# Ye-zixiao/Double-YOLO-Kaist

Measured on AMD Instinct MI355X. Metric: paired RGB+LWIR images/sec (train step), higher is better.
Workload: dtype bf16; 1 GPU; kaist_dyolov4_fshare_global_concat_se3.cfg train step (fwd+loss+bwd+Adam), 640x512 pairs, batch 16/GPU; global_batch=16, parallelism=dp1

## Files before the change

### double-yolo-kaist_amd/csrc/conv_igemm.hip

```cpp
#include <stddef.h>
#include <string.h>
#include "dyk_common.h"

int dyk_conv_launch_n128(const DykConvDesc* d, hipStream_t s);
int dyk_conv_launch_n80(const DykConvDesc* d, hipStream_t s);
int dyk_conv_launch_n160(const DykConvDesc* d, hipStream_t s);
int dyk_conv_launch_halo(const DykConvDesc* d, hipStream_t s, int th);
int dyk_conv_launch_kg(const DykConvDesc* d, hipStream_t s);
int dyk_conv_launch_lt(const DykConvDesc* d, hipStream_t s);
int dyk_conv_launch_sc(const DykConvDesc* d, hipStream_t s);
int dyk_conv_launch_pw(const DykConvDesc* d, hipStream_t s);

static int conv_validate(const DykConvDesc* d) {
    if (!d || !d->x || !d->w || !d->y) return DYK_ERR_ARG;
    if (d->ntaps < 0 || d->ntaps > DYK_MAX_TAPS) return DYK_ERR_ARG;
    if (d->B <= 0 || d->Hg <= 0 || d->Wg <= 0 || d->Cout <= 0 || d->Cin <= 0) return DYK_ERR_ARG;
    if (d->ncls < 0 || d->ncls > 4) return DYK_ERR_ARG;
    for (int c = 0; c < (d->ncls > 1 ? d->ncls : 0); ++c)
        if (d->cls_first[c] < 0 || d->cls_ntaps[c] < 0 || d->cls_first[c] + d->cls_ntaps[c] > d->ntaps || d->cls_ooy[c] < 0 ||
            d->cls_ooy[c] >= d->osy || d->cls_oox[c] < 0 || d->cls_oox[c] >= d->osx)
            return DYK_ERR_ARG;
    if (d->dtype == DYK_F16 && (d->flags & (DYK_EPI_STATS | DYK_EPI_BNFWD | DYK_EPI_BNBWD | DYK_EPI_ADDEND))) return DYK_ERR_UNSUPPORTED;
    if ((d->flags & DYK_EPI_STATS) && !d->stats) return DYK_ERR_ARG;
    if ((d->flags & DYK_EPI_RESIDUAL) && !d->res) return DYK_ERR_ARG;
    if ((d->flags & DYK_EPI_ADDEND) && (!(d->flags & DYK_EPI_BNBWD) || ((uintptr_t)d->add % 16))) return DYK_ERR_ARG;
    if (d->flags & DYK_EPI_BNFWD) {
        if (!(d->flags & DYK_EPI_STATS) || (d->flags & (DYK_EPI_AFFINE | DYK_EPI_ACCUM | DYK_EPI_OUT_F32 | DYK_EPI_BNBWD | DYK_EPI_ADDEND)))
            return DYK_ERR_ARG;
        if (d->dtype != DYK_BF16 || d->twin || d->ncls > 1 || d->bn_count <= 0) return DYK_ERR_ARG;
        if (!d->y2 || !d->bn_counter || !d->scale || !d->shift || ((uintptr_t)d->y2 % 16) || ((uintptr_t)d->bn_counter % 8)) return DYK_ERR_ARG;
        if (d->Cout % 8 || d->ldy % 8 || d->ldy2 % 8 || d->ldy2 < d->Cout) return DYK_ERR_ARG;
        if ((d->flags & DYK_EPI_RESIDUAL) && (d->ldr % 4 || ((uintptr_t)d->res % 8))) return DYK_ERR_ARG;
        if ((long)d->B * d->Ho * d->Wo * d->ldy2 >= (1L << 31)) return DYK_ERR_ARG;
    }
    if (d->flags & DYK_EPI_BNBWD) {
        if (d->flags & (DYK_EPI_AFFINE | DYK_EPI_RESIDUAL | DYK_EPI_STATS | DYK_EPI_ACCUM | DYK_EPI_OUT_F32)) return DYK_ERR_ARG;
        if (!d->res || !d->stats || !d->scale || !d->shift || !d->aux0 || !d->aux1) return DYK_ERR_ARG;
        const int es = d->dtype == DYK_F32 ? 4 : 2;
        if (d->Cout % (16 / es) || ((size_t)d->ldy * es) % 16 || ((size_t)d->ldr * es) % 16 || ((uintptr_t)d->y % 16) ||
            ((uintptr_t)d->res % 16))
            return DYK_ERR_ARG;
    }
    if (d->splitk > 1) {
        if (d->splitk > 16 || !d->sk_ws || !d->sk_cnt || ((uintptr_t)d->sk_ws % 16) || ((uintptr_t)d->sk_cnt % 4) || d->sk_cnt_n <= 0 ||
            d->sk_ws_bytes <= 0)
            return DYK_ERR_ARG;
        if (d->twin || d->ncls > 1 || (d->flags & DYK_EPI_BNFWD)) return DYK_ERR_ARG;
    }
    if (d->dtype != DYK_BF16 && d->dtype != DYK_F32 && d->dtype != DYK_F16) return DYK_ERR_ARG;
    const int epv = d->dtype == DYK_F32 ? 4 : 8;
    if (d->ldx % epv || ((uintptr_t)d->x % 16) || ((uintptr_t)d->w % 16)) return DYK_ERR_ARG;
    if ((long)d->B * d->Hi * d->Wi * d->ldx >= (1L << 31)) return DYK_ERR_ARG;
    if ((long)d->B * d->Ho * d->Wo * d->ldy >= (1L << 31)) return DYK_ERR_ARG;
    if (d->Hi > 16000 || d->Wi > 16000) return DYK_ERR_ARG;
    return DYK_OK;
}

extern "C" int dyk_conv_igemm(const DykConvDesc* d, void* stream) {
    int rc0 = conv_validate(d);
    if (rc0 != DYK_OK) return rc0;
    if (d->twin) {
        if ((rc0 = conv_validate(d->twin)) != DYK_OK) return rc0;
        const size_t lo = offsetof(DykConvDesc, dtype), hi = offsetof(DykConvDesc, twin);
        if (memcmp((const char*)d + lo, (const char*)d->twin + lo, hi - lo) != 0) return DYK_ERR_ARG;
    }
    hipStream_t s = (hipStream_t)stream;
    const int tile = d->dtype != DYK_F32 ? (d->tune >> 12) & 0xf : 0;
    if (d->flags & DYK_EPI_BNFWD) {
        if (tile == 1 || tile == 3) return dyk_conv_launch_n80(d, s);
        if (tile == 2 || tile == 4) return dyk_conv_launch_n160(d, s);
        return dyk_conv_launch_n128(d, s);
    }
    if (tile == 5) {
        const int rc = dyk_conv_launch_lt(d, s);
        if (rc != DYK_ERR_UNSUPPORTED || ((d->tune >> 23) & 1)) return rc;
        return dyk_conv_launch_n160(d, s);
    }
    if (tile == 6) {
        const int rc = (d->splitk > 1 || d->dtype != DYK_BF16) ? DYK_ERR_UNSUPPORTED : dyk_conv_launch_sc(d, s);
        if (rc != DYK_ERR_UNSUPPORTED || ((d->tune >> 23) & 1)) return rc;
        return dyk_conv_launch_n128(d, s);
    }
    if (tile == 7) {
        const int rc = dyk_conv_launch_pw(d, s);
        if (rc != DYK_ERR_UNSUPPORTED || ((d->tune >> 23) & 1)) return rc;
        return dyk_conv_launch_n128(d, s);
    }
    if (((d->tune >> 28) & 7) == 1) {
        const int rc = dyk_conv_launch_kg(d, s);
        if (rc != DYK_ERR_UNSUPPORTED || ((d->tune >> 23) & 1)) return rc;
    }
    if (tile == 3 || tile == 4) {
        const int rc = dyk_conv_launch_halo(d, s, tile == 3 ? 4 : 8);
        if (rc != DYK_ERR_UNSUPPORTED || ((d->tune >> 23) & 1)) return rc;
        return tile == 3 ? dyk_conv_launch_n80(d, s) : dyk_conv_launch_n160(d, s);
    }
    if (tile == 1) return dyk_conv_launch_n80(d, s);
    if (tile == 2) return dyk_conv_launch_n160(d, s);
    return dyk_conv_launch_n128(d, s);
}

extern "C" int dyk_conv_bnfwd_max_grid(void) { return 256; }

extern "C" int dyk_conv_grid(const DykConvDesc* d) {
    if (!d || d->B <= 0 || d->Hg <= 0 || d->Wg <= 0 || d->Cout <= 0) return DYK_ERR_ARG;
    const int tile = d->dtype != DYK_F32 ? (d->tune >> 12) & 0xf : 0;
    const int bn = (tile == 1 || tile == 3) ? 80 : ((tile == 2 || tile == 4) ? 160 : 128);
    int bm = d->Cout > 64 ? 128 : (d->Cout > 32 ? 64 : 32);
    const int bm_code = (d->tune >> 24) & 0xf;
    if (bm_code >= 1 && bm_code <= 3) bm = 16 << bm_code;
    if (bn == 80 && bm == 32) bm = 64;
    const long n = (long)d->B * d->Hg * d->Wg;
    return (int)((n + bn - 1) / bn) * ((d->Cout + bm - 1) / bm) * (d->ncls > 1 ? d->ncls : 1);
}

extern "C" int64_t dyk_conv_splitk_ws_bytes(const DykConvDesc* d, int32_t* tiles) {
    if (tiles) *tiles = 0;
    if (!d || d->B <= 0 || d->Hg <= 0 || d->Wg <= 0 || d->Cout <= 0) return DYK_ERR_ARG;
    if (d->splitk <= 1) return 0;
    const long n = (long)d->B * d->Hg * d->Wg;
    const int tile = d->dtype != DYK_F32 ? (d->tune >> 12) & 0xf : 0;
    int64_t bytes = 0;
    int32_t nt = 0;
    auto cover = [&](int bm, int bn) {
        const int64_t tm = (d->Cout + bm - 1) / bm, tn = (n + bn - 1) / bn;
        const int64_t b = tm * tn * (int64_t)d->splitk * bm * bn * 4;
        if (b > bytes) bytes = b;
        if (tm * tn > nt) nt = (int32_t)(tm * tn);
    };
    {
        const int bn = (tile == 1 || tile == 3) ? 80 : ((tile == 2 || tile == 4 || tile == 5) ? 160 : 128);
        int bm = d->Cout > 64 ? 128 : (d->Cout > 32 ? 64 : 32);
        const int bm_code = (d->tune >> 24) & 0xf;
        if (tile != 5 && bm_code >= 1 && bm_code <= 3) bm = 16 << bm_code;
        if (bn == 80 && bm == 32) bm = 64;
        if (((d->tune >> 28) & 7) == 1 && bm < 64) bm = 64;
        cover(bm, bn);
    }
    if (tile == 5) {
        const int shape = (d->tune >> 8) & 0xf;
        if (shape == 1) cover(128, 320);
        else if (shape == 2) cover(256, 160);
        else cover(128, 160);
    }
    if (tiles) *tiles = nt;
    return bytes;
}
```

### double-yolo-kaist_amd/csrc/conv_sc.hip

```cpp
#include <stddef.h>
#include <string.h>
#include <type_traits>
#include "dyk_common.h"

namespace {

#define LDS_AS __attribute__((address_space(3)))
__device__ uint4 dyk_sc_zero_page[8];

struct ScArgs {
    DykConvDesc d;
    int PH, PW, npatch;
    int miny, minx;
    int tiles_y, tiles_x, ntiles;
    int tap_shift[9];
    int tap_w[9];
    int cls_first[4], cls_ntaps[4], cls_ooy[4], cls_oox[4];
};

__device__ inline void sc_glds16(const void* gsrc, unsigned lds_addr) {
    unsigned keep;
    asm volatile("s_mov_b32 %0, m0\n\ts_mov_b32 m0, %2\n\ts_nop 0\n\tglobal_load_lds_dwordx4 %1, off\n\ts_mov_b32 m0, %0"
                 : "=&s"(keep)
                 : "v"(gsrc), "s"(lds_addr)
                 : "memory");
}
__device__ inline unsigned sc_lds_addr(const void* p) {
    return __builtin_amdgcn_readfirstlane((unsigned)(size_t)(LDS_AS const char*)p);
}

constexpr int SC_M = 32, SC_TH = 8, SC_TW = 16;

template <int NCLS, int K> struct ScCfg {
    static constexpr int PITCH = K * 2;
    static constexpr int NCH = PITCH / 16;
    static constexpr int RPI = 1024 / PITCH;
    static constexpr int R256 = PITCH >= 256 ? 1 : 256 / PITCH;
    static constexpr int PROWS = NCLS == 4 ? 9 * 17 : 10 * 18;
    static constexpr int NPI = ((PROWS + RPI - 1) / RPI + 3) / 4;
    static constexpr int P_BYTES = NPI * 4 * 1024;
    static constexpr int W_BYTES = 9 * SC_M * PITCH;
    static constexpr int NWI = W_BYTES / 1024 / 4;
    static constexpr int LDS = W_BYTES + 2 * P_BYTES + 4 * 2 * SC_M * 4 + 4 * SC_M * 4;
    static_assert(W_BYTES % 4096 == 0, "weights in whole instructions per wave");
};
template <int K> __device__ inline int sc_key(int row) { return (row / ScCfg<1, K>::R256) & (ScCfg<1, K>::NCH - 1); }

template <int NCLS, int K, int ACTB>
__global__ __launch_bounds__(256) __attribute__((amdgpu_waves_per_eu(2))) void conv_sc_kernel(const ScArgs g) {
    using C = ScCfg<NCLS, K>;
    using T = bf16_t;
    constexpr int PITCH = C::PITCH, NPI = C::NPI, NWI = C::NWI, RPI = C::RPI, VPR = C::NCH;
    const DykConvDesc& a = g.d;
    extern __shared__ __attribute__((aligned(16))) char smem[];
    char* sW = smem;
    char* sP = smem + C::W_BYTES;
    float* s_stat = (float*)(smem + C::W_BYTES + 2 * C::P_BYTES);

    const int tid = threadIdx.x, lane = tid & 63;
    const int wv = __builtin_amdgcn_readfirstlane(tid >> 6);
    const int i16 = lane & 15, kq = lane >> 4;
    const T* zero = (const T*)dyk_sc_zero_page;
    const int Hi_s = __builtin_amdgcn_readfirstlane(a.Hi), Wi_s = __builtin_amdgcn_readfirstlane(a.Wi);
    const int ldx_s = __builtin_amdgcn_readfirstlane(a.ldx), ldy_s = __builtin_amdgcn_readfirstlane(a.ldy), ldr_s = __builtin_amdgcn_readfirstlane(a.ldr);
    const int Ho_s = __builtin_amdgcn_readfirstlane(a.Ho), Wo_s = __builtin_amdgcn_readfirstlane(a.Wo);
    const int osy = __builtin_amdgcn_readfirstlane(a.osy), osx = __builtin_amdgcn_readfirstlane(a.osx);
    const int PW = g.PW;

    {
        const T* wg = (const T*)a.w;
#pragma unroll
        for (int j = 0; j < NWI; ++j) {
            const int q = j * 4 + wv;
            const int row = q * RPI + lane / VPR, ps = lane % VPR;
            const int lc = ps ^ sc_key<K>(row);
            sc_glds16(wg + (long)row * K + lc * 8, sc_lds_addr(sW + q * 1024));
        }
    }
    int p_eoff[NPI], p_yx[NPI];
#pragma unroll
    for (int j = 0; j < NPI; ++j) {
        const int row = (j * 4 + wv) * RPI + lane / VPR, ps = lane % VPR;
        const int lc = ps ^ sc_key<K>(row);
        const int py = row / PW, px = row - py * PW;
        p_yx[j] = row < g.npatch ? (py << 16) | px : (0x7000 << 16);
        p_eoff[j] = (py * Wi_s + px) * ldx_s + lc * 8;
    }
    auto stage_patch = [&](int tile, int buf) {
        const int tx = tile % g.tiles_x, r = tile / g.tiles_x;
        const int ty = r % g.tiles_y, b = r / g.tiles_y;
        const int ys = ty * SC_TH + g.miny, xs = tx * SC_TW + g.minx;
        const T* x00 = (const T*)a.x + (long)((b * Hi_s + ys) * Wi_s + xs) * ldx_s;
        char* dst = sP + buf * C::P_BYTES;
#pragma unroll
        for (int j = 0; j < NPI; ++j) {
            const int hy = p_yx[j] >> 16, hx = p_yx[j] & 0xffff;
            const bool ok = ((unsigned)(ys + hy) < (unsigned)Hi_s) & ((unsigned)(xs + hx) < (unsigned)Wi_s);
            const T* cand = x00 + p_eoff[j];
            sc_glds16(ok ? cand : zero, sc_lds_addr(dst + (j * 4 + wv) * 1024));
        }
    };

    float* s_bn = s_stat + 4 * 2 * SC_M;
    if (tid < 4 * SC_M) {
        const int which = tid / SC_M, ch = tid % SC_M;
        const float* src = which == 0 ? a.scale : which == 1 ? a.shift : which == 2 ? a.aux0 : a.aux1;
        s_bn[tid] = src[ch];
    }
    float s1[8], s2[8];
#pragma unroll
    for (int j = 0; j < 8; ++j) s1[j] = s2[j] = 0.f;
    int pb[2];
#pragma unroll
    for (int ni = 0; ni < 2; ++ni) pb[ni] = (2 * wv + ni) * PW + i16;
    int wa[2];
#pragma unroll
    for (int mi = 0; mi < 2; ++mi) wa[mi] = (mi * 16 + i16) * PITCH;
    const int wkey[2] = {sc_key<K>(i16), sc_key<K>(16 + i16)};

    int buf = 0;
    int tile = blockIdx.x;
    if (tile < g.ntiles) stage_patch(tile, 0);
    for (; tile < g.ntiles; tile += gridDim.x) {
        asm volatile("s_waitcnt vmcnt(0)" ::: "memory");
        __builtin_amdgcn_s_barrier();
        if (tile + (int)gridDim.x < g.ntiles) stage_patch(tile + gridDim.x, buf ^ 1);
        const char* P = sP + buf * C::P_BYTES;

        const int tx = tile % g.tiles_x, rr = tile / g.tiles_x;
        const int ty = rr % g.tiles_y, b = rr / g.tiles_y;
        const int xo = (tx * SC_TW + i16) * osx;
        uint2 raw[NCLS][2][2];
        int opix[NCLS][2];
#pragma unroll
        for (int c = 0; c < NCLS; ++c)
#pragma unroll
            for (int ni = 0; ni < 2; ++ni) {
                const int yo = (ty * SC_TH + 2 * wv + ni) * osy + (NCLS > 1 ? g.cls_ooy[c] : a.ooy);
                opix[c][ni] = (b * Ho_s + yo) * Wo_s + xo + (NCLS > 1 ? g.cls_oox[c] : a.oox);
#pragma unroll
                for (int mi = 0; mi < 2; ++mi)
                    raw[c][mi][ni] = *(const uint2*)((const T*)a.res + (long)opix[c][ni] * ldr_s + mi * 16 + kq * 4);
            }

        f32x4_t acc[NCLS][2][2];
#pragma unroll
        for (int c = 0; c < NCLS; ++c)
#pragma unroll
            for (int mi = 0; mi < 2; ++mi)
#pragma unroll
                for (int ni = 0; ni < 2; ++ni) acc[c][mi][ni] = (f32x4_t){0.f, 0.f, 0.f, 0.f};
        {
            int t = 0;
#pragma unroll
            for (int c = 0; c < NCLS; ++c) {
                constexpr int NT[4] = {NCLS == 4 ? 1 : 9, 2, 2, 4};
#pragma unroll
                for (int q = 0; q < NT[c]; ++q, ++t) {
                    const int shift = g.tap_shift[t];
                    const char* Wt = sW + g.tap_w[t] * (SC_M * PITCH);
                    int prow[2], pkey[2];
#pragma unroll
                    for (int ni = 0; ni < 2; ++ni) { prow[ni] = pb[ni] + shift; pkey[ni] = sc_key<K>(prow[ni]); }
#pragma unroll
                    for (int kb = 0; kb < K / 32; ++kb) {
                        const int chunk = kq + 4 * kb;
                        bf16x8_t fa[2], fb[2];
#pragma unroll
                        for (int mi = 0; mi < 2; ++mi) fa[mi] = *(const bf16x8_t*)(Wt + wa[mi] + ((chunk ^ wkey[mi]) << 4));
#pragma unroll
                        for (int ni = 0; ni < 2; ++ni) fb[ni] = *(const bf16x8_t*)(P + prow[ni] * PITCH + ((chunk ^ pkey[ni]) << 4));
#pragma unroll
                        for (int mi = 0; mi < 2; ++mi)
#pragma unroll
                            for (int ni = 0; ni < 2; ++ni)
                                acc[c][mi][ni] = __builtin_amdgcn_mfma_f32_16x16x32_bf16(fa[mi], fb[ni], acc[c][mi][ni], 0, 0, 0);
                    }
                }
            }
        }

#pragma unroll
        for (int mi = 0; mi < 2; ++mi) {
            const f32x4_t scv = *(const f32x4_t*)(s_bn + 0 * SC_M + mi * 16 + kq * 4), shv = *(const f32x4_t*)(s_bn + 1 * SC_M + mi * 16 + kq * 4);
            const f32x4_t muv = *(const f32x4_t*)(s_bn + 2 * SC_M + mi * 16 + kq * 4), rsv = *(const f32x4_t*)(s_bn + 3 * SC_M + mi * 16 + kq * 4);
#pragma unroll
            for (int c = 0; c < NCLS; ++c)
#pragma unroll
                for (int ni = 0; ni < 2; ++ni) {
                    const f32x4_t v = acc[c][mi][ni];
                    const uint32_t g01 = f32x2_to_bf16x2(v[0], v[1]), g23 = f32x2_to_bf16x2(v[2], v[3]);
                    const uint2 y2 = raw[c][mi][ni];
                    uint32_t ow[2];
#pragma unroll
                    for (int h = 0; h < 2; ++h) {
                        const uint32_t gw = h ? g23 : g01, yw = h ? y2.y : y2.x;
                        const dyk_f32x2_t gv = {__uint_as_float(gw << 16), __uint_as_float(gw & 0xffff0000u)};
                        const dyk_f32x2_t yv = {__uint_as_float(yw << 16), __uint_as_float(yw & 0xffff0000u)};
                        const int j = mi * 4 + 2 * h;
                        const dyk_f32x2_t sc2 = {scv[2 * h], scv[2 * h + 1]}, sh2 = {shv[2 * h], shv[2 * h + 1]};
                        const dyk_f32x2_t mu2 = {muv[2 * h], muv[2 * h + 1]}, rs2 = {rsv[2 * h], rsv[2 * h + 1]};
                        const dyk_f32x2_t u = yv * sc2 + sh2;
                        const dyk_f32x2_t da = gv * act_bwd2_c<ACTB>(u, a.act);
                        const dyk_f32x2_t xh = (yv - mu2) * rs2;
                        const dyk_f32x2_t p = da * xh;
                        s1[j] += da[0]; s1[j + 1] += da[1];
                        s2[j] += p[0]; s2[j + 1] += p[1];
                        ow[h] = f32x2_to_bf16x2(da[0], da[1]);
                    }
                    *(uint2*)((T*)a.y + (long)opix[c][ni] * ldy_s + mi * 16 + kq * 4) = make_uint2(ow[0], ow[1]);
                }
        }
        buf ^= 1;
    }

#pragma unroll
    for (int j = 0; j < 8; ++j) { s1[j] = row16_sum(s1[j]); s2[j] = row16_sum(s2[j]); }
    if (i16 == 0) {
#pragma unroll
        for (int mi = 0; mi < 2; ++mi)
#pragma unroll
            for (int r = 0; r < 4; ++r) {
                s_stat[(wv * 2 + 0) * SC_M + mi * 16 + kq * 4 + r] = s1[mi * 4 + r];
                s_stat[(wv * 2 + 1) * SC_M + mi * 16 + kq * 4 + r] = s2[mi * 4 + r];
            }
    }
    __syncthreads();
    if (tid < 2 * SC_M) {
        const int ml = tid % SC_M, which = tid / SC_M;
        const float tot = (s_stat[(0 * 2 + which) * SC_M + ml] + s_stat[(1 * 2 + which) * SC_M + ml]) +
                          (s_stat[(2 * 2 + which) * SC_M + ml] + s_stat[(3 * 2 + which) * SC_M + ml]);
        double* st = a.stats + (size_t)((unsigned)blockIdx.x % (unsigned)(a.stats_slots > 0 ? a.stats_slots : 1)) * 2 * a.Cout;
        atomicAdd(st + which * a.Cout + ml, (double)tot);
    }
}

bool sc_eligible(const DykConvDesc* d) {
    if (d->dtype != DYK_BF16 || d->ntaps != 9 || d->twin) return false;
    if (d->flags != DYK_EPI_BNBWD) return false;
    if (d->Cout != SC_M || (d->Cin != 64)) return false;
    if (d->isy != 1 || d->isx != 1 || d->osy != d->osx) return false;
    if (d->Hg % SC_TH || d->Wg % SC_TW) return false;
    if (d->ldx % 8 || d->ldy % 4 || d->ldr % 4 || ((uintptr_t)d->y % 8) || ((uintptr_t)d->res % 8)) return false;
    if (d->ncls > 1) {
        if (d->ncls != 4 || d->osy != 2) return false;
        if (d->Ho != 2 * d->Hg || d->Wo != 2 * d->Wg) return false;
        static const int nt[4] = {1, 2, 2, 4};
        for (int c = 0, q = 0; c < 4; q += nt[c], ++c)
            if (d->cls_ntaps[c] != nt[c] || d->cls_first[c] != q) return false;
    } else {
        if (d->osy != 1 || d->Ho != d->Hg || d->Wo != d->Wg) return false;
    }
    for (int t = 0; t < 9; ++t) {
        if (d->ncls > 1 ? (d->tdy[t] < 0 || d->tdy[t] > 1 || d->tdx[t] < 0 || d->tdx[t] > 1)
                        : (d->tdy[t] < -1 || d->tdy[t] > 1 || d->tdx[t] < -1 || d->tdx[t] > 1)) return false;
        if (d->twt[t] < 0 || d->twt[t] > 8) return false;
    }
    return true;
}

template <int NCLS, int K, int ACTB>
int sc_launch(const ScArgs& g, hipStream_t stream) {
    using C = ScCfg<NCLS, K>;
    static DykDeviceOnce attr_set;
    auto kfn = conv_sc_kernel<NCLS, K, ACTB>;
    if (attr_set.first()) {
        DYK_HIP_TRY(hipFuncSetAttribute((const void*)kfn, hipFuncAttributeMaxDynamicSharedMemorySize, (int)C::LDS));
    }
    int grid = 256 * (int)((160 * 1024) / C::LDS);
    if (grid > g.ntiles) grid = g.ntiles;
    hipLaunchKernelGGL(kfn, dim3(grid), dim3(256), C::LDS, stream, g);
    DYK_LAUNCH_CHECK();
    return DYK_OK;
}

template <int NCLS, int K>
int sc_dispatch_act(const ScArgs& g, hipStream_t s) {
    switch (g.d.act) {
    case DYK_ACT_MISH: return sc_launch<NCLS, K, DYK_ACT_MISH>(g, s);
    case DYK_ACT_LEAKY: return sc_launch<NCLS, K, DYK_ACT_LEAKY>(g, s);
    default: return sc_launch<NCLS, K, -1>(g, s);
    }
}

}

int dyk_conv_launch_sc(const DykConvDesc* d, hipStream_t s) {
    if (!sc_eligible(d)) return DYK_ERR_UNSUPPORTED;
    ScArgs g;
    g.d = *d;
    g.d.twin = nullptr;
    const int ncls = d->ncls > 1 ? 4 : 1;
    g.miny = ncls == 4 ? 0 : -1;
    g.minx = g.miny;
    g.PH = SC_TH + (ncls == 4 ? 1 : 2);
    g.PW = SC_TW + (ncls == 4 ? 1 : 2);
    g.npatch = g.PH * g.PW;
    g.tiles_y = d->Hg / SC_TH;
    g.tiles_x = d->Wg / SC_TW;
    g.ntiles = d->B * g.tiles_y * g.tiles_x;
    for (int t = 0; t < 9; ++t) {
        g.tap_shift[t] = (d->tdy[t] - g.miny) * g.PW + (d->tdx[t] - g.minx);
        g.tap_w[t] = d->twt[t];
    }
    for (int c = 0; c < 4; ++c) {
        g.cls_first[c] = ncls == 4 ? d->cls_first[c] : 0;
        g.cls_ntaps[c] = ncls == 4 ? d->cls_ntaps[c] : (c == 0 ? 9 : 0);
        g.cls_ooy[c] = ncls == 4 ? d->cls_ooy[c] : 0;
        g.cls_oox[c] = ncls == 4 ? d->cls_oox[c] : 0;
    }
    return ncls == 4 ? sc_dispatch_act<4, 64>(g, s) : sc_dispatch_act<1, 64>(g, s);
}
```

### double-yolo-kaist_amd/dyk/plan.py

```python
import ctypes
import functools
import math
import os

import torch

from . import lib as L
from .ops import conv_out_size, dgrad_classes, fwd_taps, maxpool_out_size

BN_EPS, BN_MOMENTUM = 1e-5, 0.1
HEAD_LD = 32
FWD_SLOTS_CAP = 32
FWD_SLOT_WG = 128
def _bnfwd_on():
    return os.environ.get("DYK_BNFWD", "0") != "0" and os.environ.get("DYK_PAIR", "0") == "0"


BNFWD_MAX_GRID = 256
DW_SLOTS = 32
STAT_SLOTS = 16


def _ru(n, a):
    return (n + a - 1) // a * a
# ... 1631 lines not shown
        return None
    if knob not in ("1", ""):
        return knob
    base = os.environ.get("DYK_TUNE_CACHE_DIR") or os.path.join(
        os.environ.get("XDG_CACHE_HOME") or os.path.join(os.path.expanduser("~"), ".cache"), "dyk")
    try:
        sha = L.load().dyk_build_sha().decode()
        name = torch.cuda.get_device_name(device if device is not None else torch.cuda.current_device())
    except Exception:
        return None
    name = "".join(ch if ch.isalnum() else "_" for ch in name)
    knobs = "".join("%s=%s;" % (k, os.environ[k]) for k in sorted(os.environ) if k.startswith(_TUNE_KNOBS) and k not in (
        "DYK_TUNE_CACHE", "DYK_TUNE_CACHE_DIR", "DYK_TUNE_VERBOSE"))
    import hashlib
    tag = hashlib.sha1(knobs.encode()).hexdigest()[:8] if knobs else "default"
    return os.path.join(base, "tune_%s_%s_%s.json" % (sha, name, tag))


def _tune_cache_load():
    if _TUNE_FILE["loaded"]:
        return
    _TUNE_FILE["loaded"] = True
    path = _TUNE_FILE["path"] = _tune_file_path()
    if not path or not os.path.exists(path):
        return
    import json
    try:
        with open(path) as f:
            data = json.load(f)
    except (OSError, ValueError):
        return
    import ast
    for k, (best, ms) in data.items():
        key = ast.literal_eval(k)
        if key not in _TUNE_CACHE:
            _TUNE_CACHE[key] = tuple(best) if isinstance(best, list) else best
            if ms is not None:
                _TUNE_MS[key] = ms


def _tune_cache_save():
    path = _TUNE_FILE["path"]
    if not path:
        return
    import json
    data = {}
    if os.path.exists(path):
        try:
            with open(path) as f:
                data = json.load(f)
        except (OSError, ValueError):
            data = {}
    for key, best in _TUNE_CACHE.items():
        data.setdefault(repr(key), [list(best) if isinstance(best, tuple) else best, _TUNE_MS.get(key)])
    try:
        os.makedirs(os.path.dirname(path), exist_ok=True)
        tmp = "%s.%d.tmp" % (path, os.getpid())
        with open(tmp, "w") as f:
            json.dump(data, f)
        os.replace(tmp, path)
    except OSError:
        pass


_H16 = (L.DYK_BF16, L.DYK_F16)


def pw_eligible(d):
    if d.dtype == L.DYK_F16 and d.flags != 0:
        return False
    if d.dtype not in _H16 or d.ntaps != 1 or d.tdy[0] or d.tdx[0] or d.ncls > 1 or d.twin or d.splitk > 1:
        return False
    if (d.isy, d.isx, d.osy, d.osx, d.ooy, d.oox) != (1, 1, 1, 1, 0, 0):
        return False
    if not (d.Hg == d.Hi == d.Ho and d.Wg == d.Wi == d.Wo):
        return False
    if d.flags not in (0, L.EPI_STATS, L.EPI_BNBWD, L.EPI_BNBWD | L.EPI_ADDEND):
        return False
    if not (d.flags & L.EPI_BNBWD) and d.act != L.ACT_CODES["linear"]:
        return False
    return d.Cin % 32 == 0 and d.Cin <= 256 and d.Cout % 8 == 0 and d.ldx % 8 == 0 and d.ldy % 8 == 0


def _conv_candidates(d):
    es = 2 if d.dtype in _H16 else 4
    bkbs = [64] + ([128] if (d.Cin * es) % 128 == 0 else [])
    tiles = [0, 1, 2] if d.dtype in _H16 else [0]
    if (d.dtype in _H16 and d.ntaps == 9 and d.isy == 1 and d.osy == 1 and d.Hg == d.Hi and d.Wg == d.Wi
            and d.Wi % 20 == 0 and d.Hi % 4 == 0):
        tiles += [3] + ([4] if d.Hi % 8 == 0 else [])
    bms = [0] + ([2] if d.Cout > 64 else ([1] if d.Cout > 32 else []))
    out = []
    for bkb in bkbs:
        for pipe in (2, 3, 4, 6):
            for t in tiles:
                for bm in bms:
                    if t in (1, 3, 4) and bm == 1:
                        continue
                    if t in (3, 4) and pipe != 2:
                        continue
                    out.append(bkb | (pipe << 8) | (t << 12) | (bm << 24))
    if (d.dtype in _H16 and d.ntaps == 9 and d.isy == 1 and d.osy == 1 and d.Hg == d.Hi and d.Wg == d.Wi and d.ncls <= 1
            and d.Cin % 32 == 0 and d.Wi % 20 == 0 and not (d.flags & (L.EPI_OUT_F32 | L.EPI_BNFWD))
            and os.environ.get("DYK_CONV_LT", "1") != "0"):
        for shape in (1, 2, 3):
            if shape == 2 and d.Cout < 256:
                continue
            out.append((5 << 12) | (shape << 8))
    if (d.dtype == L.DYK_BF16 and d.ntaps == 9 and d.Cout == 32 and d.Cin == 64 and d.flags == L.EPI_BNBWD and d.isy == 1
            and d.Hg % 8 == 0 and d.Wg % 16 == 0 and os.environ.get("DYK_CONV_SC", "1") != "0"):
        out.append(6 << 12)
    if pw_eligible(d) and os.environ.get("DYK_CONV_PW", "1") != "0":
        for nxs in (2, 3, 4):
            out.append((7 << 12) | (nxs << 8))
            if d.Cout <= 64:
                out.append((7 << 12) | (nxs << 8) | (1 << 24))
            else:
                out.append((7 << 12) | (nxs << 8) | (1 << 25))
    if d.dtype in _H16 and (d.Cin * es) % 128 == 0 and d.Cin >= 128 and os.environ.get("DYK_CONV_KG", "1") != "0":
        for t in (1, 2):
            for bm in bms:
                if bm != 1:
                    out.append(128 | (2 << 8) | (t << 12) | (bm << 24) | (1 << 28))
    return out


def _conv_split_candidates(d):
    if os.environ.get("DYK_CONV_SPLITK", "1") == "0":
        return []
    if d.twin or d.ncls > 1 or d.flags & L.EPI_BNFWD:
        return []
    es = 2 if d.dtype in _H16 else 4
    npix = d.B * d.Hg * d.Wg
    max_s = 8
    out = []

    def splits(tiles, kchunks):
        return [s for s in (2, 3, 4, 6, 8) if s <= max_s and tiles * s <= 640 and tiles * (s - 1) < 512 and kchunks // s >= 2]
    if (d.Cin * es) % 64:
        return []
    bkbs = [128] if (d.Cin * es) % 128 == 0 else [64]
    tiles_px = [(2, 160), (0, 128), (1, 80)] if d.dtype in _H16 else [(0, 128)]
    bms = [(0, 128 if d.Cout > 64 else (64 if d.Cout > 32 else 32))] + ([(2, 64)] if d.Cout > 64 else [])
    for bkb in bkbs:
        kch = (d.Cin * es) // bkb
        for t, bn in tiles_px:
            for bmc, bm in bms:
                if t == 1 and bm < 64:
                    continue
                tiles = -(-npix // bn) * -(-d.Cout // bm)
                for s in splits(tiles, kch):
                    for pipe in (2, 3):
                        out.append((bkb | (pipe << 8) | (t << 12) | (bmc << 24), s))
                    if d.dtype in _H16 and bkb == 128 and t in (1, 2) and bm >= 64 and kch // s >= 4 and os.environ.get("DYK_CONV_KG", "1") != "0":
                        out.append((128 | (2 << 8) | (t << 12) | (bmc << 24) | (1 << 28), s))
    if (d.dtype in _H16 and d.ntaps == 9 and d.isy == 1 and d.osy == 1 and d.Hg == d.Hi and d.Wg == d.Wi
            and d.Cin % 32 == 0 and d.Wi % 20 == 0 and not (d.flags & L.EPI_OUT_F32) and os.environ.get("DYK_CONV_LT", "1") != "0"):
        for shape, (bm, bn, kg) in ((1, (128, 320, 1)), (2, (256, 160, 1)), (3, (128, 160, 2))):
            if shape == 2 and d.Cout < 256:
                continue
            if npix % bn:
                continue
            tiles = (npix // bn) * -(-d.Cout // bm)
            for s in splits(tiles, (d.Cin // 32) // kg):
                out.append(((5 << 12) | (shape << 8), s))
    return out


WGRAD_KG1, WGRAD_KG2 = 1 << 8, 2 << 8
WGRAD_CAP64 = 1 << 24
WGRAD_MT = 1 << 28
WGRAD_RB = 2 << 28
WGRAD_PS = 3 << 28
WGRAD_PS_CAP64, WGRAD_PS_STAGE64 = 1 << 8, 1 << 12
WGRAD_EXCLUSIVE = 1 << 20


def wgrad_variant(tune):
    return (tune >> 28) & 7


_WGRAD_CANDIDATES = [2, 3, 2 | WGRAD_KG2, 2 | WGRAD_CAP64, 3 | WGRAD_CAP64, 2 | WGRAD_KG2 | WGRAD_CAP64, 2 | WGRAD_MT]
if os.environ.get("DYK_WGRAD_RB", "1") != "0":
    _WGRAD_CANDIDATES.append(2 | WGRAD_KG1 | WGRAD_RB | WGRAD_EXCLUSIVE)
if os.environ.get("DYK_WGRAD_PS", "1") != "0":
    _WGRAD_CANDIDATES += [WGRAD_PS | 2 | WGRAD_EXCLUSIVE, WGRAD_PS | 3 | WGRAD_EXCLUSIVE,
                          WGRAD_PS | 4 | WGRAD_PS_CAP64 | WGRAD_EXCLUSIVE, WGRAD_PS | 4 | WGRAD_PS_CAP64 | WGRAD_PS_STAGE64 | WGRAD_EXCLUSIVE]


def _time_launch(fn, desc, stream, reps=3):
    e0, e1 = torch.cuda.Event(enable_timing=True), torch.cuda.Event(enable_timing=True)
    L.check(fn(ctypes.byref(desc), stream), "autotune launch")
    e0.record()
    for _ in range(reps):
# ... 199 lines not shown
```

### double-yolo-kaist_amd/dyk/twins.py

```python
import ctypes
import heapq

from . import lib as L
from .plan import wgrad_variant

_IMG = ("image",)


def _section_signature(md):
    skip = {"layers", "from", "type"}
    items = []
    for k in sorted(md):
        if k in skip:
            continue
        v = md[k]
        try:
            v = tuple(v.reshape(-1).tolist()) if hasattr(v, "reshape") else (tuple(v) if isinstance(v, (list, tuple)) else v)
        except Exception:
            v = str(v)
        items.append((k, v))
    return (md["type"], tuple(items))


def section_inputs(defs, mods, second):
    out = []
    for i, md in enumerate(defs):
        t = md["type"]
        if t == "route":
            out.append([int(q) for q in mods[i].layers])
        elif t == "shortcut":
            out.append([i - 1] + [int(q) for q in mods[i].layers])
        elif i == 0 or (second is not None and i == second):
            out.append([_IMG])
        else:
            out.append([i - 1])
    return out


def twin_layers(defs, mods, second):
    if second is None:
        return {}
    inputs = section_inputs(defs, mods, second)
    h, alias = [], set()
    for i, md in enumerate(defs):
        if md["type"] == "route" and len(inputs[i]) == 1:
            h.append(h[inputs[i][0]])
            alias.add(i)
            continue
        key = (_section_signature(md), tuple(_IMG if q is _IMG else h[q] for q in inputs[i]))
        h.append(hash(key))
    groups = {}
    for i, v in enumerate(h):
        if i not in alias:
            groups.setdefault(v, []).append(i)
    twins = {}
    for g in groups.values():
        if len(g) % 2 == 0:
            m = len(g) // 2
            for k in range(m):
                twins[g[k]], twins[g[k + m]] = g[k + m], g[k]
    return twins


def _bytes(d, cls, first, last):
    lo, hi = getattr(cls, first).offset, getattr(cls, last).offset
    return ctypes.string_at(ctypes.addressof(d) + lo, hi - lo)


def _nulls(d, names):
    return tuple(bool(getattr(d, n)) for n in names)


_EW_PTRS = ("a", "b", "out", "p0", "p1", "p2", "p3", "red", "aux", "aux2")
_FIN_PTRS = ("stats", "gamma", "beta", "running_mean", "running_var", "scale", "shift", "save_mean", "save_rstd")


def pair_signature(op, d, plan):
    if op == L.OP_CONV:
        if d.flags & L.EPI_BNFWD:
            return None
        if d.splitk > 1:
            return None
        if ((d.tune >> 12) & 0xf) == 7:
            return None
        if ((d.tune >> 12) & 0xf) == 6:
            return None
        return (op, _bytes(d, L.DykConvDesc, "dtype", "twin"), _nulls(d, ("scale", "shift", "res", "stats", "aux0", "aux1", "add")))
    if op == L.OP_WGRAD:
        if wgrad_variant(d.tune) in (2, 3):
            return None
        return (op, _bytes(d, L.DykWgradDesc, "part_stride", "twin"), bool(d.part))
    if op in (L.OP_BN_ACT_FWD, L.OP_BN_BWD_REDUCE, L.OP_BN_BWD_APPLY, L.OP_AXPBY):
        return (op, _bytes(d, L.DykEwDesc, "dtype", "twin"), _nulls(d, _EW_PTRS))
    if op == L.OP_BN_FINALIZE:
        return (op, _bytes(d, L.DykBnFinalizeDesc, "C", "twin"), _nulls(d, _FIN_PTRS))
    if op == L.OP_BN_FWD_FUSED:
        f = plan._desc_at[d.p[0]]
        a = plan._desc_at[d.p[1]]
        return (op, _bytes(f, L.DykBnFinalizeDesc, "C", "twin"), _nulls(f, _FIN_PTRS),
                _bytes(a, L.DykEwDesc, "dtype", "twin"), _nulls(a, _EW_PTRS))
    return None


def ancestors(deps):
    anc = []
    for i, dl in enumerate(deps):
        m = 0
        for j in dl:
            m |= anc[j] | (1 << j)
        anc.append(m)
    return anc


def worth_pairing(op, d, plan, mode, max_bytes):
    if mode == "all":
        return True
    if mode != "ew" or op in (L.OP_CONV, L.OP_WGRAD):
        return False
    e = plan._desc_at[d.p[1]] if op == L.OP_BN_FWD_FUSED else d
    if op == L.OP_BN_FINALIZE:
        return True
    es = 2 if e.dtype in (L.DYK_BF16, L.DYK_F16) else 4
    return float(e.npix) * e.C * es <= max_bytes


def find_pairs(cmds, deps, layer_of, twin_of, plan, mode="ew", max_bytes=48e6):
    buckets = {}
    for i, (op, d) in enumerate(cmds):
        l = layer_of[i]
        t = twin_of.get(l)
        if t is None:
            continue
        sig = pair_signature(op, d, plan)
        if sig is None or not worth_pairing(op, d, plan, mode, max_bytes):
            continue
        lo, side = (l, 0) if l < t else (t, 1)
        buckets.setdefault((lo, sig), ([], []))[side].append(i)
    anc = ancestors(deps)
    pairs = []
    for (lo, sig), (A, B) in buckets.items():
        if len(A) != len(B):
            continue
        for a, b in zip(A, B):
            i, j = (a, b) if a < b else (b, a)
            if (anc[j] >> i) & 1:
                continue
            pairs.append((i, j))
    pairs.sort()
    return pairs


def merge(n, deps, costs, pairs, pair_cost=0.8):
    pairs = list(pairs)
    while True:
        node_of = list(range(n))
        for (i, j) in pairs:
            node_of[j] = i
        nd = {}
        for i in range(n):
            k = node_of[i]
            s = nd.setdefault(k, set())
            for j in deps[i]:
                if node_of[j] != k:
                    s.add(node_of[j])
        users = {k: [] for k in nd}
        missing = {}
# ... 34 lines not shown
```

Before: 601.0 pairs/s.

## Add resident-filter 3x3 conv kernel and extend SC kernel to multiple Cout tiles

Adds a new conv kernel variant (tile code 8) for 3x3 bf16 convolutions with small Cin. It keeps a 64-channel weight slice resident in LDS while persistent walkers stream double-buffered input patches via direct global-to-LDS loads, and it fuses BN statistics accumulation. The autotuner gets it as a candidate, and twin pairing excludes it. The SC backward kernel is also generalized to split Cout across blocks, which covers the Cout=64/Cin=128 four-class case with lower occupancy. This adds autotuner search options and more kernel code paths, and the resident-filter design depends on the persistent-grid sizing.

```diff
diff --git a/double-yolo-kaist_amd/csrc/conv_igemm.hip b/double-yolo-kaist_amd/csrc/conv_igemm.hip
--- a/double-yolo-kaist_amd/csrc/conv_igemm.hip
+++ b/double-yolo-kaist_amd/csrc/conv_igemm.hip
@@ -10,6 +10,7 @@
 int dyk_conv_launch_lt(const DykConvDesc* d, hipStream_t s);
 int dyk_conv_launch_sc(const DykConvDesc* d, hipStream_t s);
 int dyk_conv_launch_pw(const DykConvDesc* d, hipStream_t s);
+int dyk_conv_launch_rf(const DykConvDesc* d, hipStream_t s);
 
 static int conv_validate(const DykConvDesc* d) {
     if (!d || !d->x || !d->w || !d->y) return DYK_ERR_ARG;
@@ -86,6 +87,11 @@
         if (rc != DYK_ERR_UNSUPPORTED || ((d->tune >> 23) & 1)) return rc;
         return dyk_conv_launch_n128(d, s);
     }
+    if (tile == 8) {
+        const int rc = dyk_conv_launch_rf(d, s);
+        if (rc != DYK_ERR_UNSUPPORTED || ((d->tune >> 23) & 1)) return rc;
+        return dyk_conv_launch_n128(d, s);
+    }
     if (((d->tune >> 28) & 7) == 1) {
         const int rc = dyk_conv_launch_kg(d, s);
         if (rc != DYK_ERR_UNSUPPORTED || ((d->tune >> 23) & 1)) return rc;
diff --git a/double-yolo-kaist_amd/csrc/conv_rf.hip b/double-yolo-kaist_amd/csrc/conv_rf.hip
--- /dev/null
+++ b/double-yolo-kaist_amd/csrc/conv_rf.hip
@@ -0,0 +1,264 @@
+#include <stddef.h>
+#include <string.h>
+#include "dyk_common.h"
+
+namespace {
+
+#define LDS_AS __attribute__((address_space(3)))
+__device__ uint4 dyk_rf_zero_page[8];
+
+struct RfArgs {
+    DykConvDesc d;
+    int npatch;
+    int tiles_y, tiles_x, ntiles;
+    int nct;
+    int xcd;
+    int tap_shift[9];
+};
+
+__device__ inline void rf_glds16(const void* gsrc, unsigned lds_addr) {
+    unsigned keep;
+    asm volatile("s_mov_b32 %0, m0\n\ts_mov_b32 m0, %2\n\ts_nop 0\n\tglobal_load_lds_dwordx4 %1, off\n\ts_mov_b32 m0, %0"
+                 : "=&s"(keep)
+                 : "v"(gsrc), "s"(lds_addr)
+                 : "memory");
+}
+__device__ inline unsigned rf_lds_addr(const void* p) {
+    return __builtin_amdgcn_readfirstlane((unsigned)(size_t)(LDS_AS const char*)p);
+}
+
+constexpr int RF_M = 64, RF_TW = 16;
+
+template <int S, int K, int NI> struct RfCfg {
+    static constexpr int TH = 4 * NI;
+    static constexpr int PH = S * (TH - 1) + 3, PW = S * (RF_TW - 1) + 3;
+    static constexpr int PWE = S == 2 ? RF_TW + 1 : PW;
+    static constexpr int PITCH = K * 2;
+    static constexpr int NCH = PITCH / 16;
+    static constexpr int RPI = 1024 / PITCH;
+    static constexpr int R256 = 256 / PITCH;
+    static constexpr int PROWS = PH * PW;
+    static constexpr int NPI = ((PROWS + RPI - 1) / RPI + 3) / 4;
+    static constexpr int P_BYTES = NPI * 4 * 1024;
+    static constexpr int W_BYTES = 9 * RF_M * PITCH;
+    static constexpr int NWI = W_BYTES / 1024 / 4;
+    static constexpr int NST = 4 * NI;
+    static constexpr int LDS = W_BYTES + 2 * P_BYTES + 4 * 2 * RF_M * 4;
+    static_assert(W_BYTES % 4096 == 0, "weights in whole instructions per wave");
+    static_assert(RF_M % RPI == 0, "the rows of a weight DMA instruction share a tap");
+    static_assert(LDS <= 160 * 1024, "weights + two patches in LDS");
+};
+template <int K> __device__ inline int rf_key(int row) { return (row / (256 / (K * 2))) & (K / 8 - 1); }
+
+template <int S, int K, int NI>
+__global__ __launch_bounds__(256) __attribute__((amdgpu_waves_per_eu(2))) void conv_rf_kernel(const RfArgs g) {
+    using C = RfCfg<S, K, NI>;
+    using T = bf16_t;
+    constexpr int PITCH = C::PITCH, NPI = C::NPI, NWI = C::NWI, RPI = C::RPI, VPR = C::NCH, PW = C::PW, TH = C::TH;
+    const DykConvDesc& a = g.d;
+    extern __shared__ __attribute__((aligned(16))) char smem[];
+    char* sW = smem;
+    char* sP = smem + C::W_BYTES;
+    float* s_stat = (float*)(smem + C::W_BYTES + 2 * C::P_BYTES);
+
+    const int tid = threadIdx.x, lane = tid & 63;
+    const int wv = __builtin_amdgcn_readfirstlane(tid >> 6);
+    const int i16 = lane & 15, kq = lane >> 4;
+    const T* zero = (const T*)dyk_rf_zero_page;
+    const int Hi_s = __builtin_amdgcn_readfirstlane(a.Hi), Wi_s = __builtin_amdgcn_readfirstlane(a.Wi);
+    const int ldx_s = __builtin_amdgcn_readfirstlane(a.ldx), ldy_s = __builtin_amdgcn_readfirstlane(a.ldy);
+    const int Ho_s = __builtin_amdgcn_readfirstlane(a.Ho), Wo_s = __builtin_amdgcn_readfirstlane(a.Wo);
+    const int Cout_s = __builtin_amdgcn_readfirstlane(a.Cout);
+    const int tiles_x = __builtin_amdgcn_readfirstlane(g.tiles_x), tiles_y = __builtin_amdgcn_readfirstlane(g.tiles_y);
+    const int ntiles = __builtin_amdgcn_readfirstlane(g.ntiles);
+
+    const int nct = __builtin_amdgcn_readfirstlane(g.nct);
+    const int bx = blockIdx.x;
+    int ct, wi;
+    if (g.xcd) { ct = (bx >> 3) % nct; wi = ((bx >> 3) / nct) * 8 + (bx & 7); }
+    else { ct = bx % nct; wi = bx / nct; }
+    const int nwalk = (int)gridDim.x / nct;
+    const int m0 = ct * RF_M;
+
+    {
+        const T* wg = (const T*)a.w;
+#pragma unroll
+        for (int j = 0; j < NWI; ++j) {
+            const int q = j * 4 + wv;
+            const int row = q * RPI + lane / VPR, ps = lane % VPR;
+            const int lc = ps ^ rf_key<K>(row);
+            const long srow = (long)(row >> 6) * Cout_s + m0 + (row & 63);
+            rf_glds16(wg + srow * K + lc * 8, rf_lds_addr(sW + q * 1024));
+        }
+    }
+    int p_eoff[NPI], p_yx[NPI];
+#pragma unroll
+    for (int j = 0; j < NPI; ++j) {
+        const int row = (j * 4 + wv) * RPI + lane / VPR, ps = lane % VPR;
+        const int lc = ps ^ rf_key<K>(row);
+        const int py = row / PW, q = row - py * PW;
+        const int px = S == 2 ? (q < C::PWE ? 2 * q : 2 * (q - C::PWE) + 1) : q;
+        p_yx[j] = row < g.npatch ? (py << 16) | px : (0x7000 << 16);
+        p_eoff[j] = (py * Wi_s + px) * ldx_s + lc * 8;
+    }
+    auto stage_patch = [&](int tile, int buf) {
+        const int tx = tile % tiles_x, r = tile / tiles_x;
+        const int ty = r % tiles_y, b = r / tiles_y;
+        const int ys = ty * TH * S - 1, xs = tx * RF_TW * S - 1;
+        const T* x00 = (const T*)a.x + (long)((b * Hi_s + ys) * Wi_s + xs) * ldx_s;
+        char* dst = sP + buf * C::P_BYTES;
+#pragma unroll
+        for (int j = 0; j < NPI; ++j) {
+            const int hy = p_yx[j] >> 16, hx = p_yx[j] & 0xffff;
+            const bool ok = ((unsigned)(ys + hy) < (unsigned)Hi_s) & ((unsigned)(xs + hx) < (unsigned)Wi_s);
+            const T* cand = x00 + p_eoff[j];
+            rf_glds16(ok ? cand : zero, rf_lds_addr(dst + (j * 4 + wv) * 1024));
+        }
+    };
+
+    float s1[16], s2[16];
+#pragma unroll
+    for (int j = 0; j < 16; ++j) s1[j] = s2[j] = 0.f;
+    int pb[NI];
+#pragma unroll
+    for (int ni = 0; ni < NI; ++ni) pb[ni] = S * (NI * wv + ni) * PW + i16;
+    int wa[4], wkey[4];
+#pragma unroll
+    for (int mi = 0; mi < 4; ++mi) { wa[mi] = (mi * 16 + i16) * PITCH; wkey[mi] = rf_key<K>(mi * 16 + i16); }
+
+    int buf = 0;
+    bool first = true;
+    int tile = wi;
+    if (tile < ntiles) stage_patch(tile, 0);
+    for (; tile < ntiles; tile += nwalk) {
+        if (first) asm volatile("s_waitcnt vmcnt(0)" ::: "memory");
+        else asm volatile("s_waitcnt vmcnt(%0)" ::"n"(C::NST) : "memory");
+        first = false;
+        __builtin_amdgcn_s_barrier();
+        if (tile + nwalk < ntiles) stage_patch(tile + nwalk, buf ^ 1);
+        const char* P = sP + buf * C::P_BYTES;
+
+        f32x4_t acc[4][NI];
+#pragma unroll
+        for (int mi = 0; mi < 4; ++mi)
+#pragma unroll
+            for (int ni = 0; ni < NI; ++ni) acc[mi][ni] = (f32x4_t){0.f, 0.f, 0.f, 0.f};
+#pragma unroll
+        for (int kb = 0; kb < K / 32; ++kb) {
+            const int chunk = kq + 4 * kb;
+#pragma unroll
+            for (int t = 0; t < 9; ++t) {
+                const char* Wt = sW + t * (RF_M * PITCH);
+                bf16x8_t fa[4], fb[NI];
+#pragma unroll
+                for (int mi = 0; mi < 4; ++mi) fa[mi] = *(const bf16x8_t*)(Wt + wa[mi] + ((chunk ^ wkey[mi]) << 4));
+#pragma unroll
+                for (int ni = 0; ni < NI; ++ni) {
+                    const int prow = pb[ni] + g.tap_shift[t];
+                    fb[ni] = *(const bf16x8_t*)(P + prow * PITCH + ((chunk ^ rf_key<K>(prow)) << 4));
+                }
+#pragma unroll
+                for (int mi = 0; mi < 4; ++mi)
+#pragma unroll
+                    for (int ni = 0; ni < NI; ++ni)
+                        acc[mi][ni] = __builtin_amdgcn_mfma_f32_16x16x32_bf16(fa[mi], fb[ni], acc[mi][ni], 0, 0, 0);
+            }
+        }
+
+        const int tx = tile % tiles_x, rr = tile / tiles_x;
+        const int ty = rr % tiles_y, b = rr / tiles_y;
+        const int xo = tx * RF_TW + i16;
+#pragma unroll
+        for (int ni = 0; ni < NI; ++ni) {
+            const int yo = ty * TH + NI * wv + ni;
+            T* yp = (T*)a.y + (long)((b * Ho_s + yo) * Wo_s + xo) * ldy_s + m0 + kq * 4;
+#pragma unroll
+            for (int mi = 0; mi < 4; ++mi) {
+                const f32x4_t v = acc[mi][ni];
+#pragma unroll
+                for (int r = 0; r < 4; ++r) { s1[mi * 4 + r] += v[r]; s2[mi * 4 + r] += v[r] * v[r]; }
+                *(uint2*)(yp + mi * 16) = make_uint2(f32x2_to_bf16x2(v[0], v[1]), f32x2_to_bf16x2(v[2], v[3]));
+            }
+        }
+        buf ^= 1;
+    }
+
+#pragma unroll
+    for (int j = 0; j < 16; ++j) { s1[j] = row16_sum(s1[j]); s2[j] = row16_sum(s2[j]); }
+    if (i16 == 0) {
+#pragma unroll
+        for (int mi = 0; mi < 4; ++mi)
+#pragma unroll
+            for (int r = 0; r < 4; ++r) {
+                s_stat[(wv * 2 + 0) * RF_M + mi * 16 + kq * 4 + r] = s1[mi * 4 + r];
+                s_stat[(wv * 2 + 1) * RF_M + mi * 16 + kq * 4 + r] = s2[mi * 4 + r];
+            }
+    }
+    __syncthreads();
+    if (tid < 2 * RF_M) {
+        const int ml = tid % RF_M, which = tid / RF_M;
+        const float tot = (s_stat[(0 * 2 + which) * RF_M + ml] + s_stat[(1 * 2 + which) * RF_M + ml]) +
+                          (s_stat[(2 * 2 + which) * RF_M + ml] + s_stat[(3 * 2 + which) * RF_M + ml]);
+        double* st = a.stats + (size_t)((unsigned)blockIdx.x % (unsigned)(a.stats_slots > 0 ? a.stats_slots : 1)) * 2 * a.Cout;
+        atomicAdd(st + which * a.Cout + m0 + ml, (double)tot);
+    }
+}
+
+constexpr int rf_ni(int stride) { return stride == 1 ? 2 : 1; }
+
+bool rf_eligible(const DykConvDesc* d) {
+    if (d->dtype != DYK_BF16 || d->ntaps != 9 || d->twin || d->splitk > 1 || d->ncls > 1) return false;
+    if (d->flags != DYK_EPI_STATS || !d->stats) return false;
+    if (d->Cin != 32 && d->Cin != 64) return false;
+    if (d->Cout % RF_M) return false;
+    if (d->isy != d->isx || (d->isy != 1 && d->isy != 2)) return false;
+    if (d->isy == 2 && d->Cin != 32) return false;
+    if (d->osy != 1 || d->osx != 1 || d->ooy || d->oox || d->Ho != d->Hg || d->Wo != d->Wg) return false;
+    if (d->Hg % (4 * rf_ni(d->isy)) || d->Wg % RF_TW) return false;
+    if (d->ldx % 8 || d->ldy % 8 || ((uintptr_t)d->y % 16) || d->ldx < d->Cin || d->ldy < d->Cout) return false;
+    for (int t = 0; t < 9; ++t) {
+        if (d->tdy[t] < -1 || d->tdy[t] > 1 || d->tdx[t] < -1 || d->tdx[t] > 1) return false;
+        if (d->twt[t] != t) return false;
+    }
+    return true;
+}
+
+template <int S, int K, int NI>
+int rf_launch(RfArgs& g, hipStream_t stream) {
+    using C = RfCfg<S, K, NI>;
+    static DykDeviceOnce attr_set;
+    auto kfn = conv_rf_kernel<S, K, NI>;
+    if (attr_set.first()) {
+        DYK_HIP_TRY(hipFuncSetAttribute((const void*)kfn, hipFuncAttributeMaxDynamicSharedMemorySize, (int)C::LDS));
+    }
+    const DykConvDesc& d = g.d;
+    g.npatch = C::PROWS;
+    g.tiles_y = d.Hg / C::TH;
+    g.tiles_x = d.Wg / RF_TW;
+    g.ntiles = d.B * g.tiles_y * g.tiles_x;
+    g.nct = d.Cout / RF_M;
+    for (int t = 0; t < 9; ++t) {
+        const int dy = d.tdy[t] + 1, dx = d.tdx[t] + 1;
+        g.tap_shift[t] = dy * C::PW + (S == 2 ? (dx == 1 ? C::PWE : dx / 2) : dx);
+    }
+    int walkers = 256 * (int)((160 * 1024) / C::LDS) / g.nct;
+    const int cap = (d.tune >> 8) & 0xf;
+    if (cap > 0 && walkers > cap) walkers = cap;
+    if (walkers > g.ntiles) walkers = g.ntiles;
+    if (walkers < 1) walkers = 1;
+    g.xcd = walkers % 8 == 0 && g.nct > 1;
+    hipLaunchKernelGGL(kfn, dim3(walkers * g.nct), dim3(256), C::LDS, stream, g);
+    DYK_LAUNCH_CHECK();
+    return DYK_OK;
+}
+
+}
+
+int dyk_conv_launch_rf(const DykConvDesc* d, hipStream_t s) {
+    if (!rf_eligible(d)) return DYK_ERR_UNSUPPORTED;
+    RfArgs g;
+    g.d = *d;
+    g.d.twin = nullptr;
+    if (d->isy == 1) return d->Cin == 32 ? rf_launch<1, 32, rf_ni(1)>(g, s) : rf_launch<1, 64, rf_ni(1)>(g, s);
+    return rf_launch<2, 32, rf_ni(2)>(g, s);
+}
diff --git a/double-yolo-kaist_amd/csrc/conv_sc.hip b/double-yolo-kaist_amd/csrc/conv_sc.hip
--- a/double-yolo-kaist_amd/csrc/conv_sc.hip
+++ b/double-yolo-kaist_amd/csrc/conv_sc.hip
@@ -13,6 +13,7 @@
     int PH, PW, npatch;
     int miny, minx;
     int tiles_y, tiles_x, ntiles;
+    int nct;
     int tap_shift[9];
     int tap_w[9];
     int cls_first[4], cls_ntaps[4], cls_ooy[4], cls_oox[4];
@@ -47,7 +48,7 @@
 template <int K> __device__ inline int sc_key(int row) { return (row / ScCfg<1, K>::R256) & (ScCfg<1, K>::NCH - 1); }
 
 template <int NCLS, int K, int ACTB>
-__global__ __launch_bounds__(256) __attribute__((amdgpu_waves_per_eu(2))) void conv_sc_kernel(const ScArgs g) {
+__global__ __launch_bounds__(256) __attribute__((amdgpu_waves_per_eu(K == 128 ? 1 : 2))) void conv_sc_kernel(const ScArgs g) {
     using C = ScCfg<NCLS, K>;
     using T = bf16_t;
     constexpr int PITCH = C::PITCH, NPI = C::NPI, NWI = C::NWI, RPI = C::RPI, VPR = C::NCH;
@@ -66,15 +67,19 @@
     const int Ho_s = __builtin_amdgcn_readfirstlane(a.Ho), Wo_s = __builtin_amdgcn_readfirstlane(a.Wo);
     const int osy = __builtin_amdgcn_readfirstlane(a.osy), osx = __builtin_amdgcn_readfirstlane(a.osx);
     const int PW = g.PW;
+    const int nct = __builtin_amdgcn_readfirstlane(g.nct);
+    const int m0 = ((int)blockIdx.x % nct) * SC_M;
+    const int walker = (int)blockIdx.x / nct, nwalk = (int)gridDim.x / nct;
 
     {
-        const T* wg = (const T*)a.w;
+        const T* wg = (const T*)a.w + (long)m0 * K;
+        const int Cout_s = __builtin_amdgcn_readfirstlane(a.Cout);
 #pragma unroll
         for (int j = 0; j < NWI; ++j) {
             const int q = j * 4 + wv;
             const int row = q * RPI + lane / VPR, ps = lane % VPR;
             const int lc = ps ^ sc_key<K>(row);
-            sc_glds16(wg + (long)row * K + lc * 8, sc_lds_addr(sW + q * 1024));
+            sc_glds16(wg + ((long)(row / SC_M) * Cout_s + row % SC_M) * K + lc * 8, sc_lds_addr(sW + q * 1024));
         }
     }
     int p_eoff[NPI], p_yx[NPI];
@@ -105,7 +110,7 @@
     if (tid < 4 * SC_M) {
         const int which = tid / SC_M, ch = tid % SC_M;
         const float* src = which == 0 ? a.scale : which == 1 ? a.shift : which == 2 ? a.aux0 : a.aux1;
-        s_bn[tid] = src[ch];
+        s_bn[tid] = src[m0 + ch];
     }
     float s1[8], s2[8];
 #pragma unroll
@@ -119,12 +124,12 @@
     const int wkey[2] = {sc_key<K>(i16), sc_key<K>(16 + i16)};
 
     int buf = 0;
-    int tile = blockIdx.x;
+    int tile = walker;
     if (tile < g.ntiles) stage_patch(tile, 0);
-    for (; tile < g.ntiles; tile += gridDim.x) {
+    for (; tile < g.ntiles; tile += nwalk) {
         asm volatile("s_waitcnt vmcnt(0)" ::: "memory");
         __builtin_amdgcn_s_barrier();
-        if (tile + (int)gridDim.x < g.ntiles) stage_patch(tile + gridDim.x, buf ^ 1);
+        if (tile + nwalk < g.ntiles) stage_patch(tile + nwalk, buf ^ 1);
         const char* P = sP + buf * C::P_BYTES;
 
         const int tx = tile % g.tiles_x, rr = tile / g.tiles_x;
@@ -140,7 +145,7 @@
                 opix[c][ni] = (b * Ho_s + yo) * Wo_s + xo + (NCLS > 1 ? g.cls_oox[c] : a.oox);
 #pragma unroll
                 for (int mi = 0; mi < 2; ++mi)
-                    raw[c][mi][ni] = *(const uint2*)((const T*)a.res + (long)opix[c][ni] * ldr_s + mi * 16 + kq * 4);
+                    raw[c][mi][ni] = *(const uint2*)((const T*)a.res + (long)opix[c][ni] * ldr_s + m0 + mi * 16 + kq * 4);
             }
 
         f32x4_t acc[NCLS][2][2];
@@ -208,7 +213,7 @@
                         s2[j] += p[0]; s2[j + 1] += p[1];
                         ow[h] = f32x2_to_bf16x2(da[0], da[1]);
                     }
-                    *(uint2*)((T*)a.y + (long)opix[c][ni] * ldy_s + mi * 16 + kq * 4) = make_uint2(ow[0], ow[1]);
+                    *(uint2*)((T*)a.y + (long)opix[c][ni] * ldy_s + m0 + mi * 16 + kq * 4) = make_uint2(ow[0], ow[1]);
                 }
         }
         buf ^= 1;
@@ -231,14 +236,14 @@
         const float tot = (s_stat[(0 * 2 + which) * SC_M + ml] + s_stat[(1 * 2 + which) * SC_M + ml]) +
                           (s_stat[(2 * 2 + which) * SC_M + ml] + s_stat[(3 * 2 + which) * SC_M + ml]);
         double* st = a.stats + (size_t)((unsigned)blockIdx.x % (unsigned)(a.stats_slots > 0 ? a.stats_slots : 1)) * 2 * a.Cout;
-        atomicAdd(st + which * a.Cout + ml, (double)tot);
+        atomicAdd(st + which * a.Cout + m0 + ml, (double)tot);
     }
 }
 
 bool sc_eligible(const DykConvDesc* d) {
     if (d->dtype != DYK_BF16 || d->ntaps != 9 || d->twin) return false;
     if (d->flags != DYK_EPI_BNBWD) return false;
-    if (d->Cout != SC_M || (d->Cin != 64)) return false;
+    if (!((d->Cout == SC_M && d->Cin == 64) || (d->Cout == 2 * SC_M && d->Cin == 128 && d->ncls == 4))) return false;
     if (d->isy != 1 || d->isx != 1 || d->osy != d->osx) return false;
     if (d->Hg % SC_TH || d->Wg % SC_TW) return false;
     if (d->ldx % 8 || d->ldy % 4 || d->ldr % 4 || ((uintptr_t)d->y % 8) || ((uintptr_t)d->res % 8)) return false;
@@ -267,9 +272,9 @@
     if (attr_set.first()) {
         DYK_HIP_TRY(hipFuncSetAttribute((const void*)kfn, hipFuncAttributeMaxDynamicSharedMemorySize, (int)C::LDS));
     }
-    int grid = 256 * (int)((160 * 1024) / C::LDS);
-    if (grid > g.ntiles) grid = g.ntiles;
-    hipLaunchKernelGGL(kfn, dim3(grid), dim3(256), C::LDS, stream, g);
+    int walkers = 256 * (int)((160 * 1024) / C::LDS) / g.nct;
+    if (walkers > g.ntiles) walkers = g.ntiles;
+    hipLaunchKernelGGL(kfn, dim3(walkers * g.nct), dim3(256), C::LDS, stream, g);
     DYK_LAUNCH_CHECK();
     return DYK_OK;
 }
@@ -299,6 +304,7 @@
     g.tiles_y = d->Hg / SC_TH;
     g.tiles_x = d->Wg / SC_TW;
     g.ntiles = d->B * g.tiles_y * g.tiles_x;
+    g.nct = d->Cout / SC_M;
     for (int t = 0; t < 9; ++t) {
         g.tap_shift[t] = (d->tdy[t] - g.miny) * g.PW + (d->tdx[t] - g.minx);
         g.tap_w[t] = d->twt[t];
@@ -309,5 +315,6 @@
         g.cls_ooy[c] = ncls == 4 ? d->cls_ooy[c] : 0;
         g.cls_oox[c] = ncls == 4 ? d->cls_oox[c] : 0;
     }
+    if (d->Cin == 128) return sc_dispatch_act<4, 128>(g, s);
     return ncls == 4 ? sc_dispatch_act<4, 64>(g, s) : sc_dispatch_act<1, 64>(g, s);
 }
diff --git a/double-yolo-kaist_amd/dyk/plan.py b/double-yolo-kaist_amd/dyk/plan.py
--- a/double-yolo-kaist_amd/dyk/plan.py
+++ b/double-yolo-kaist_amd/dyk/plan.py
@@ -1737,6 +1737,20 @@
     return d.Cin % 32 == 0 and d.Cin <= 256 and d.Cout % 8 == 0 and d.ldx % 8 == 0 and d.ldy % 8 == 0
 
 
+def rf_eligible(d):
+    if d.dtype != L.DYK_BF16 or d.ntaps != 9 or d.twin or d.splitk > 1 or d.ncls > 1:
+        return False
+    if d.flags != L.EPI_STATS or d.Cin not in (32, 64) or d.Cout % 64:
+        return False
+    if d.isy != d.isx or d.isy not in (1, 2) or (d.isy == 2 and d.Cin != 32) or (d.osy, d.osx, d.ooy, d.oox) != (1, 1, 0, 0):
+        return False
+    if d.Ho != d.Hg or d.Wo != d.Wg or d.Hg % (8 if d.isy == 1 else 4) or d.Wg % 16:
+        return False
+    if d.ldx % 8 or d.ldy % 8 or d.ldx < d.Cin or d.ldy < d.Cout:
+        return False
+    return all(-1 <= d.tdy[t] <= 1 and -1 <= d.tdx[t] <= 1 and d.twt[t] == t for t in range(9))
+
+
 def _conv_candidates(d):
     es = 2 if d.dtype in _H16 else 4
     bkbs = [64] + ([128] if (d.Cin * es) % 128 == 0 else [])
@@ -1762,9 +1776,11 @@
             if shape == 2 and d.Cout < 256:
                 continue
             out.append((5 << 12) | (shape << 8))
-    if (d.dtype == L.DYK_BF16 and d.ntaps == 9 and d.Cout == 32 and d.Cin == 64 and d.flags == L.EPI_BNBWD and d.isy == 1
-            and d.Hg % 8 == 0 and d.Wg % 16 == 0 and os.environ.get("DYK_CONV_SC", "1") != "0"):
+    if (d.dtype == L.DYK_BF16 and d.ntaps == 9 and ((d.Cout, d.Cin) == (32, 64) or ((d.Cout, d.Cin) == (64, 128) and d.ncls == 4))
+            and d.flags == L.EPI_BNBWD and d.isy == 1 and d.Hg % 8 == 0 and d.Wg % 16 == 0 and os.environ.get("DYK_CONV_SC", "1") != "0"):
         out.append(6 << 12)
+    if rf_eligible(d) and os.environ.get("DYK_CONV_RF", "1") != "0":
+        out.append(8 << 12)
     if pw_eligible(d) and os.environ.get("DYK_CONV_PW", "1") != "0":
         for nxs in (2, 3, 4):
             out.append((7 << 12) | (nxs << 8))
diff --git a/double-yolo-kaist_amd/dyk/twins.py b/double-yolo-kaist_amd/dyk/twins.py
--- a/double-yolo-kaist_amd/dyk/twins.py
+++ b/double-yolo-kaist_amd/dyk/twins.py
@@ -82,6 +82,8 @@
         if d.splitk > 1:
             return None
         if ((d.tune >> 12) & 0xf) == 7:
+            return None
+        if ((d.tune >> 12) & 0xf) == 8:
             return None
         if ((d.tune >> 12) & 0xf) == 6:
             return None
```

Result: no change. 598.7 pairs/s (-0.4%).
